# whaiproject/BetaZero

Measured on AMD Instinct MI355X. Metric: selfplay_games_per_s, higher is better.
Workload: dtype bf16

## Files before the change

betazero_amd/_lib.py:

```python
import ctypes as C
import os

HERE = os.path.dirname(os.path.abspath(__file__))
SO = os.environ.get("BZ_HIP_SO") or os.path.join(HERE, "libbz_hip.so")
ABI_VERSION = 7

BZ_OK, BZ_EINVAL, BZ_EILLEGAL_MOVE, BZ_EHIP, BZ_ENOMEM, BZ_ENOGPU, BZ_ESTATE = range(7)
GAME_TTT, GAME_REVERSI, GAME_REVERSI6, GAME_REVERSI4 = 0, 1, 2, 3
EVAL_UNIFORM, EVAL_HASH, EVAL_NET_F32, EVAL_NET_BF16, EVAL_EXTERNAL, EVAL_NET_FP8, EVAL_MLP_F32, EVAL_MLP_BF16 = range(8)
ST_RUNNING, ST_TERMINAL, ST_ILLEGAL, ST_MUST_PASS = range(4)
PASS_ACTION = 64
ENGINE_REUSE_SUBTREE = 1
ENGINE_EVAL_CACHE = 2
ENGINE_EVAL_CACHE_CARRY = 4
ENGINE_LEAVES_SHIFT = 8
ENGINE_LEAVES_MASK = 31 << ENGINE_LEAVES_SHIFT
PROBE_OPS = ("expf_spec", "logf_spec", "tanhf_spec", "fsqrt", "fdiv", "u01_spec", "hash_logit", "hash_value", "gamma_spec")
PROBE_HOST, PROBE_DEVICE = 0, 1
PROBE_MAP, PROBE_SWEEP = 0, 1
PROF_SLOTS = ("tower", "stem", "heads", "select", "expand_backup", "search_fused", "play", "env_step")
COUNTER_NAMES = ("n_sims", "n_path_nodes", "n_child_scored", "n_edges_backed", "n_expanded",
                 "n_child_written", "n_env_steps", "n_net_leaves", "n_cache_hits", "n_cache_hits_prev", "n_collisions")

u64, u32, i32, i64, vp = C.c_uint64, C.c_uint32, C.c_int32, C.c_int64, C.c_void_p
# ... 85 lines not shown
    "bz_ttt_step_batch": (i32, [vp, vp, vp, vp, i64, vp, vp, vp, vp, vp, vp]),
    "bz_reversi_minimax": (i32, [u64, u64, i32, i32, C.POINTER(i32), C.POINTER(i32)]),
    "bz_ttt_minimax": (i32, [u32, u32, i32, C.POINTER(i32), C.POINTER(i32)]),
    "bz_reversi_minimax_batch": (i32, [vp, vp, vp, i64, i32, i32, vp, vp, vp]),
    "bz_ttt_minimax_batch": (i32, [vp, vp, vp, vp, i64, vp, vp, vp]),
    "bz_augment_d4_batch": (i32, [vp, vp, vp, i64, i32, i32, vp, vp, vp, vp, vp]),
    "bz_net_update": (i32, [vp, vp, vp]),
    "bz_net_param_count": (i64, [i32, i32, i32]),
    "bz_net_workspace_bytes": (i64, [i32, i32, i32, i32]),
    "bz_net_create": (i32, [i32, i32, i32, i32, vp, vp, i64, vp, C.POINTER(vp)]),
    "bz_net_destroy": (i32, [vp]),
    "bz_net_forward_f32": (i32, [vp, vp, vp, i32, vp, vp, vp]),
    "bz_net_forward_bf16": (i32, [vp, vp, vp, i32, vp, vp, vp]),
    "bz_net_forward_fp8": (i32, [vp, vp, vp, i32, vp, vp, vp]),
    "bz_sym_index": (u32, [u64, u64, u64]),
    "bz_sym_board": (i32, [u64, i32, i32, C.POINTER(u64)]),
    "bz_sym_action_map": (i32, [i32, i32, vp]),
    "bz_net_sym_scratch_bytes": (i64, [i64]),
    "bz_net_forward_sym": (i32, [vp, i32, vp, vp, i32, i32, i32, u64, vp, i64, vp, vp, vp]),
    "bz_net_forward_sym_counted": (i32, [vp, i32, vp, vp, i32, vp, i32, i32, u64, vp, vp, vp]),
    "bz_net_forward_counted": (i32, [vp, i32, vp, vp, i32, vp, vp, vp, vp]),
    "bz_net_set_adaptive_shape": (i32, [vp, i32]),
    "bz_net_shape_tally": (i32, [vp, vp, vp]),
    "bz_mlp_param_count": (i64, [i32]),
    "bz_mlp_workspace_bytes": (i64, [i32, i32]),
    "bz_mlp_create": (i32, [i32, i32, vp, vp, i64, vp, C.POINTER(vp)]),
    "bz_mlp_destroy": (i32, [vp]),
    "bz_mlp_update": (i32, [vp, vp, vp]),
    "bz_mlp_forward_f32": (i32, [vp, vp, vp, i32, vp, vp]),
    "bz_mlp_forward_bf16": (i32, [vp, vp, vp, i32, vp, vp]),
    "bz_mlp_forward_states_f32": (i32, [vp, vp, i32, vp, vp]),
    "bz_mlp_forward_states_bf16": (i32, [vp, vp, i32, vp, vp]),
    "bz_mlp_train_workspace_bytes": (i64, [i32, i32]),
    "bz_mlp_train_step": (i32, [vp, vp, vp, vp, vp, vp, vp, vp, i32, C.POINTER(MlpAdam), vp, i64, vp, vp, vp, vp]),
    "bz_engine_workspace_bytes": (i64, [C.POINTER(EngineCfg)]),
    "bz_engine_create": (i32, [C.POINTER(EngineCfg), vp, i64, C.POINTER(vp)]),
    "bz_engine_destroy": (i32, [vp]),
    "bz_engine_get_layout": (i32, [vp, C.POINTER(EngineLayout)]),
    "bz_engine_set_net": (i32, [vp, vp]),
    "bz_engine_set_mlp": (i32, [vp, vp]),
    "bz_engine_debug_set_search_seq": (i32, [vp, C.c_uint32]),
    "bz_engine_set_eval_symmetry": (i32, [vp, i32, u64]),
    "bz_engine_reset_games": (i32, [vp, vp]),
    "bz_engine_set_roots": (i32, [vp, vp, vp, vp, vp]),
    "bz_engine_search": (i32, [vp, vp]),
    "bz_engine_root_begin": (i32, [vp, vp]),
# ... 181 lines not shown
```

betazero_amd/csrc/bz_net.hip:

```cpp
#include <limits.h>
#include <math.h>
#include <stdlib.h>
#include <new>
#include <atomic>
#include <vector>

#include "bz_common.h"
#include "bz_math.h"
#include "bz_sym.h"
#include "bz_tower.h"

using namespace bz;

using namespace bz_tower;

struct bz_net {
    int C, NB, VH, max_batch;
    float *stem_w, *stem_b;
    float *conv_w, *conv_b;
    __bf16* conv_wf;
    __bf16 *stem_wf, *head_wf;
    __bf16 *conv_wf16, *stem_wf16;
    uint8_t *conv_wf8, *head_wf8;
    float *dq8, *head_dq8, *ones;
    float *pol_w, *pol_b, *polfc_wT, *polfc_b;
    float *val_w, *val_b, *v1_wT, *v1_b, *v2_w, *v2_b;
    float *act_a, *act_b;
    void* ws_base;
    hipEvent_t f32_done;
    bool f32_used;
    int adaptive;
    uint32_t* tally;
    uint64_t epoch;
};

namespace {

#define BZ_NET_SYM 0
#include "bz_net_ends_body.h"
#undef BZ_NET_SYM
#define BZ_NET_SYM 1
#include "bz_net_ends_body.h"
#undef BZ_NET_SYM

__global__ void __launch_bounds__(256) k_conv_f32(const float* __restrict__ in, const float* __restrict__ w,
                                                  const float* __restrict__ b, const float* skip, float* out, int n,
                                                  const u32* n_dev, int C) {
    extern __shared__ __attribute__((aligned(16))) char smem_raw[];
    float* xs = reinterpret_cast<float*>(smem_raw);
    int pos = blockIdx.x;
    if (n_dev) n = (int)*n_dev;
    if (pos >= n) return;
    const float* xin = in + (size_t)pos * 64 * C;
    for (int i = threadIdx.x; i < 64 * C; i += 256) xs[i] = xin[i];
// ... 14 lines not shown
            }
            const float* wt = w + (size_t)t * C * C + co;
            for (int ci = 0; ci < C; ++ci) {
                float wv = wt[(size_t)ci * C];
#pragma unroll
                for (int j = 0; j < 8; ++j)
                    if (src[j] >= 0) acc[j] = __builtin_fmaf(xs[src[j] + ci], wv, acc[j]);
            }
        }
#pragma unroll
        for (int j = 0; j < 8; ++j) {
            size_t o = ((size_t)pos * 64 + c0 + j) * C + co;
            float v = acc[j];
            if (skip) v = v + skip[o];
            out[o] = relu_f32(v);
        }
    }
}

typedef Tw<64, 2> TwS64;
typedef Tw<128, 1> TwS128;
typedef Tw<256, 1> TwS256;
typedef Tw<128, 4, true> TwM16;
constexpr int kSmallBatch = 256;
constexpr int kAdaptT1 = 256;
enum { kShapeLatency = 0, kShapeMiddle = 1, kShapeThroughput = 2, kShapes = 4 };

struct TowerArgs {
    const u64 *own, *opp;
    const u32* n_dev;
    int n, n_layers, VH;
    int lo, hi;
    u32* tally;
    const uint4* wf;
    const uint4 *wf16, *stem_wf16;
    const float* bias;
    const uint4* stem_wf;
    const float* stem_b;
    const uint4* head_wf;
    const uint4 *wf8, *head_wf8;
    const float *dq8, *head_dq8, *ones;
    const float *pol_b, *val_b;
    const float *polfc_wT, *polfc_b;
    const float *v1_wT, *v1_b, *v2_w, *v2_b;
    float *logits, *value;
};
// ... 27 lines not shown
    unsigned wd[4];
#pragma unroll
    for (int j = 0; j < 4; ++j) {
        const int t = 4 * g + j;
        const int bit = t <= 8 ? (t / 3) * 8 + t % 3 : 31;
        const unsigned o = (n_own >> bit) & 1u, p = (n_opp >> bit) & 1u;
        wd[j] = (o | (p << 16)) * 0x3F80u;
    }
    uint4 u = make_uint4(wd[0], wd[1], wd[2], wd[3]);
    return __builtin_bit_cast(bf16x8, u);
}

__device__ __forceinline__ float wave_sum(float x) {
#pragma unroll
    for (int o = 32; o > 0; o >>= 1) x += __shfl_xor(x, o, 64);
    return x;
}

#define BZ_NET_SYM 0
#include "bz_net_tower_bf16_body.h"
#undef BZ_NET_SYM
#define BZ_NET_SYM 1
#include "bz_net_tower_bf16_body.h"
#undef BZ_NET_SYM

namespace f8 {
typedef int v8i __attribute__((ext_vector_type(8)));
typedef int v4i __attribute__((ext_vector_type(4)));
constexpr int kCell = 128, kRowC = 9;
constexpr int kTile = (8 * kRowC + 1) * kCell;
constexpr int kBuf = 4 * kTile;
constexpr int kLds = 2 * kBuf;
constexpr float kActScale = 16.0f;
constexpr int kUnit = 0x7F7F7F7F;

__device__ __forceinline__ constexpr int cell_at(int y, int x) { return (y * kRowC + x + 1) * kCell; }
__device__ __forceinline__ int sw3(int p, int x) { return ((x & 7) >> 1) | ((p & 1) << 2); }
template <int DX>
__device__ __forceinline__ int tap_off(int r, int h) {
    const int xx = (r & 7) + DX;
    return (r >> 3) * kTile + cell_at(0, xx) + (((2 * h) ^ sw3(r >> 3, xx)) << 4);
}
__device__ __forceinline__ v8i ld32(const char* p0, int off, int imm) {
    v4i lo = *reinterpret_cast<const v4i*>(p0 + off + imm);
    v4i hi = *reinterpret_cast<const v4i*>(p0 + (off ^ 16) + imm);
    v8i v = {lo[0], lo[1], lo[2], lo[3], hi[0], hi[1], hi[2], hi[3]};
// ... 381 lines not shown
BZ_EXPORT int32_t bz_net_create(int32_t C, int32_t NB, int32_t VH, int32_t max_batch, const float* p, void* ws,
                                int64_t bytes, void* stream, bz_net** out) {
    BZ_REQUIRE(shape_ok(C, NB, VH, max_batch) && p && ws && out, "bz_net_create: unsupported shape or null pointer");
    if (bz_device_count() <= 0) { set_error("bz_net_create: no HIP device (the net has no CPU path)"); return BZ_ENOGPU; }
    NetOffsets o = net_carve(C, NB, VH, max_batch);
    if (bytes < o.total) { set_error("bz_net_create: workspace too small"); return BZ_ENOMEM; }
    BZ_REQUIRE((reinterpret_cast<uintptr_t>(ws) & 255) == 0, "bz_net_create: workspace must be 256-byte aligned");
    bz_net* n = new (std::nothrow) bz_net();
    if (!n) { set_error("out of host memory"); return BZ_ENOMEM; }
    n->C = C; n->NB = NB; n->VH = VH; n->max_batch = max_batch;
    n->stem_w = at<float>(ws, o.stem_w); n->stem_b = at<float>(ws, o.stem_b);
    n->conv_w = at<float>(ws, o.conv_w); n->conv_b = at<float>(ws, o.conv_b);
    n->conv_wf = (C == 64 || C == 128 || C == 256) ? at<__bf16>(ws, o.conv_wf) : nullptr;
    n->stem_wf = at<__bf16>(ws, o.stem_wf); n->head_wf = at<__bf16>(ws, o.head_wf);
    n->conv_wf16 = C == kTC ? at<__bf16>(ws, o.conv_wf16) : nullptr; n->stem_wf16 = C == kTC ? at<__bf16>(ws, o.stem_wf16) : nullptr;
    n->conv_wf8 = C == kTC ? at<uint8_t>(ws, o.conv_wf8) : nullptr; n->head_wf8 = at<uint8_t>(ws, o.head_wf8);
    n->dq8 = at<float>(ws, o.dq8); n->head_dq8 = at<float>(ws, o.head_dq8); n->ones = at<float>(ws, o.ones);
    n->pol_w = at<float>(ws, o.pol_w); n->pol_b = at<float>(ws, o.pol_b);
    n->polfc_wT = at<float>(ws, o.polfc_wT); n->polfc_b = at<float>(ws, o.polfc_b);
    n->val_w = at<float>(ws, o.val_w); n->val_b = at<float>(ws, o.val_b);
    n->v1_wT = at<float>(ws, o.v1_wT); n->v1_b = at<float>(ws, o.v1_b);
    n->v2_w = at<float>(ws, o.v2_w); n->v2_b = at<float>(ws, o.v2_b);
    n->act_a = at<float>(ws, o.act_a); n->act_b = at<float>(ws, o.act_b);
    n->tally = at<uint32_t>(ws, o.tally); n->adaptive = 1;

    n->ws_base = ws;
    n->f32_used = false;
    if (hipEventCreateWithFlags(&n->f32_done, hipEventDisableTiming) != hipSuccess) {
        delete n; set_error("bz_net_create: hipEventCreate failed"); return BZ_EHIP;
    }
    if (hipMemsetAsync(n->tally, 0, kShapes * sizeof(uint32_t), (hipStream_t)stream) != hipSuccess) {
        (void)hipEventDestroy(n->f32_done); delete n; set_error("bz_net_create: hipMemsetAsync failed"); return BZ_EHIP;
    }
    int32_t urc = upload_params(n, p, (hipStream_t)stream);
    if (urc != BZ_OK) { delete n; return urc; }
    {
        hipError_t e3 = hipSuccess;
#define BZ_TOWER_LDS(GEOM) hipFuncSetAttribute(reinterpret_cast<const void*>(k_tower_bf16<GEOM>), hipFuncAttributeMaxDynamicSharedMemorySize, GEOM::LDS)
        if (C == 64) { e3 = BZ_TOWER_LDS(Tw<64>); if (e3 == hipSuccess) e3 = BZ_TOWER_LDS(TwS64); }
        if (C == 128) { e3 = BZ_TOWER_LDS(TwM16); if (e3 == hipSuccess) e3 = BZ_TOWER_LDS(TwS128); }
        if (C == 256) { e3 = BZ_TOWER_LDS(Tw<256>); if (e3 == hipSuccess) e3 = BZ_TOWER_LDS(TwS256); }
#undef BZ_TOWER_LDS
        if (e3 != hipSuccess) { delete n; return hip_fail(e3, "hipFuncSetAttribute(k_tower_bf16)"); }
#define BZ_TOWER_LDS(GEOM) hipFuncSetAttribute(reinterpret_cast<const void*>(k_sym_bf16<GEOM>), hipFuncAttributeMaxDynamicSharedMemorySize, GEOM::LDS)
        if (C == 64) { e3 = BZ_TOWER_LDS(Tw<64>); if (e3 == hipSuccess) e3 = BZ_TOWER_LDS(TwS64); }
        if (C == 128) { e3 = BZ_TOWER_LDS(TwM16); if (e3 == hipSuccess) e3 = BZ_TOWER_LDS(TwS128); }
        if (C == 256) { e3 = BZ_TOWER_LDS(Tw<256>); if (e3 == hipSuccess) e3 = BZ_TOWER_LDS(TwS256); }
#undef BZ_TOWER_LDS
        if (e3 != hipSuccess) { delete n; return hip_fail(e3, "hipFuncSetAttribute(k_sym_bf16)"); }
        if (C == 256) {
            e3 = hipFuncSetAttribute(reinterpret_cast<const void*>(k_heads<float>), hipFuncAttributeMaxDynamicSharedMemorySize,
                                     (int)((64 * (C + 1) + 128 + 64 + 64) * sizeof(float)));
            if (e3 == hipSuccess)
                e3 = hipFuncSetAttribute(reinterpret_cast<const void*>(k_sym_heads<float>), hipFuncAttributeMaxDynamicSharedMemorySize,
                                         (int)((64 * (C + 1) + 128 + 64 + 64) * sizeof(float)));
            if (e3 == hipSuccess)
                e3 = hipFuncSetAttribute(reinterpret_cast<const void*>(k_conv_f32), hipFuncAttributeMaxDynamicSharedMemorySize,
                                         (int)(64 * C * sizeof(float)));
            if (e3 != hipSuccess) { delete n; return hip_fail(e3, "hipFuncSetAttribute(f32 parity kernels)"); }
        }
    }
    if (C == kTC) {
        hipError_t e3 = hipFuncSetAttribute(reinterpret_cast<const void*>(f8::k_tower_fp8), hipFuncAttributeMaxDynamicSharedMemorySize,
                                 f8::kLds);
        if (e3 == hipSuccess)
            e3 = hipFuncSetAttribute(reinterpret_cast<const void*>(f8::k_sym_fp8), hipFuncAttributeMaxDynamicSharedMemorySize, f8::kLds);
        if (e3 != hipSuccess) { delete n; return hip_fail(e3, "hipFuncSetAttribute(k_tower_fp8)"); }
    }
    *out = n;
    return BZ_OK;
}

// ... 62 lines not shown
    T.dq8 = n->dq8; T.head_dq8 = n->head_dq8; T.ones = n->ones;
    T.polfc_wT = n->polfc_wT; T.polfc_b = n->polfc_b; T.v1_wT = n->v1_wT; T.v1_b = n->v1_b; T.v2_w = n->v2_w;
    T.v2_b = n->v2_b; T.logits = logits; T.value = value;
    T.lo = 0; T.hi = INT_MAX; T.tally = nullptr;
    {
        ProfScope ps(BZ_PROF_TOWER, stream);
        const bool small = cnt <= kSmallBatch;
        const bool dev128 = n_dev && !small && n->C == 128 && !fp8;
        const int mode = dev128 ? n->adaptive : 0;
        TowerArgs TS = T;
        if (dev128) T.tally = n->tally + kShapeThroughput;
        if (mode == 1) { TS.n = kAdaptT1 < cnt ? kAdaptT1 : cnt; TS.hi = kAdaptT1; TS.tally = n->tally + kShapeLatency; T.lo = kAdaptT1 + 1; }
        if (mode == 2) T.tally = n->tally + kShapeLatency;
#define BZ_TOWER_LAUNCH(KERNEL, GEOM, TA, ...) hipLaunchKernelGGL(KERNEL<GEOM>, dim3((TA.n + GEOM::P - 1) / GEOM::P), dim3(256), GEOM::LDS, s, TA, ##__VA_ARGS__)
#define BZ_TOWER_PICK(KERNEL, ...) do {                                                                               \
            if (n->C == 64) { if (small) BZ_TOWER_LAUNCH(KERNEL, TwS64, T, ##__VA_ARGS__); else BZ_TOWER_LAUNCH(KERNEL, Tw<64>, T, ##__VA_ARGS__); }        \
            else if (n->C == 256) { if (small) BZ_TOWER_LAUNCH(KERNEL, TwS256, T, ##__VA_ARGS__); else BZ_TOWER_LAUNCH(KERNEL, Tw<256>, T, ##__VA_ARGS__); } \
            else if (mode == 1) { BZ_TOWER_LAUNCH(KERNEL, TwS128, TS, ##__VA_ARGS__); BZ_TOWER_LAUNCH(KERNEL, TwM16, T, ##__VA_ARGS__); }                    \
            else { if (small || mode == 2) BZ_TOWER_LAUNCH(KERNEL, TwS128, T, ##__VA_ARGS__); else BZ_TOWER_LAUNCH(KERNEL, TwM16, T, ##__VA_ARGS__); }       \
        } while (0)
        if (fp8 && Y) hipLaunchKernelGGL(f8::k_sym_fp8, dim3((cnt + 3) / 4), dim3(256), f8::kLds, s, T, *Y);
        else if (fp8) hipLaunchKernelGGL(f8::k_tower_fp8, dim3((cnt + 3) / 4), dim3(256), f8::kLds, s, T);
        else if (Y) BZ_TOWER_PICK(k_sym_bf16, *Y);
        else BZ_TOWER_PICK(k_tower_bf16);
#undef BZ_TOWER_PICK
#undef BZ_TOWER_LAUNCH
    }
    BZ_LAUNCH_CHECK("k_tower_bf16");
    return BZ_OK;
}

BZ_EXPORT int32_t bz_net_set_adaptive_shape(bz_net* n, int32_t mode) {
    BZ_REQUIRE(n && mode >= 0 && mode <= 2, "bz_net_set_adaptive_shape: null net, or mode not 0 (off), 1 (on) or 2 (latency shape always)");
    n->adaptive = mode;
    return BZ_OK;
}
BZ_EXPORT int32_t bz_net_shape_tally(bz_net* n, int64_t* counts, void* stream) {
    BZ_REQUIRE(n && counts, "bz_net_shape_tally: null pointer");
    uint32_t h[kShapes];
    BZ_HIP(hipMemcpyAsync(h, n->tally, sizeof(h), hipMemcpyDeviceToHost, (hipStream_t)stream));
    BZ_HIP(hipMemsetAsync(n->tally, 0, sizeof(h), (hipStream_t)stream));
    BZ_HIP(hipStreamSynchronize((hipStream_t)stream));
    for (int i = 0; i < 3; ++i) counts[i] = h[i];
    return BZ_OK;
}

uint64_t bz_net_epoch(const bz_net* n) { return n ? n->epoch : 0; }
int32_t bz_net_max_batch(const bz_net* n) { return n ? n->max_batch : 0; }

int32_t bz_net_forward_dev(bz_net* n, int bf16 , const uint64_t* own, const uint64_t* opp, int32_t max_n,
                           const uint32_t* n_dev, float* logits, float* value, void* stream) {
    BZ_REQUIRE(n && own && opp && logits && value, "bz_net_forward: null pointer");
    BZ_REQUIRE(bf16 != 1 || n->C == 64 || n->C == 128 || n->C == 256,
               "bz_net_forward_bf16: the MFMA tower is built for 64, 128 or 256 channels");
    BZ_REQUIRE(bf16 != 2 || n->C == kTC, "bz_net_forward_fp8: the fp8 tower is built for C == 128");
    BZ_REQUIRE(max_n >= 0 && max_n <= n->max_batch, "bz_net_forward: batch exceeds max_batch");
    if (max_n == 0) return BZ_OK;
// ... 84 lines not shown
```

betazero_amd/csrc/bz_net_tower_bf16_body.h:

```cpp

template <class G>
__global__ void __launch_bounds__(256, 1)
#if BZ_NET_SYM
k_sym_bf16(TowerArgs T, bz_sym::Args Y) {
#else
k_tower_bf16(TowerArgs T) {
#endif
    constexpr int C = G::C, P = G::P, PW = G::PW, MW = G::MW;
    extern __shared__ __attribute__((aligned(16))) char smem[];
    const int tid = threadIdx.x, lane = tid & 63;
    const int w = __builtin_amdgcn_readfirstlane(tid >> 6);
    const int pos0 = blockIdx.x * P;
    if (T.n_dev) T.n = (int)*T.n_dev;
    if (pos0 >= T.n || T.n < T.lo || T.n > T.hi) return;
    if (T.tally && blockIdx.x == 0 && tid == 0) atomicAdd(T.tally, 1u);
    [[maybe_unused]] unsigned long long tacc[4] = {0, 0, 0, 0}, tk0 = 0, tk1 = 0, tr0 = 0, tr1 = 0;
    BZ_STAMP(tk0);
#ifdef BZ_EXP_STAMPS
    tr0 = __builtin_amdgcn_s_memrealtime();
#endif
    char* bufX = smem;
    char* bufM = smem + G::BUF;
    const int r = lane & 31, h = lane >> 5;

    constexpr int ZC = G::CELL / 16;
    for (int i = tid; i < 2 * P * 9 * ZC; i += 256) {
        int k = i % ZC, j = (i / ZC) % 9, pb = i / (9 * ZC);
        *reinterpret_cast<uint4*>(smem + pb * G::TILE + j * G::ROWC * G::CELL + k * 16) = make_uint4(0, 0, 0, 0);
    }
    const int wt0 = G::wt0(w), wp0 = G::pos0(w);
    const uint4* ap = G::M16 ? T.wf16 + (size_t)wt0 * 2 * 64 : T.wf + (size_t)wt0 * 64;
    typename WSetsOf<G>::type WS;
    if constexpr (G::M16) {
#pragma unroll
        for (int kq = 0; kq < G::KQ; ++kq)
#pragma unroll
            for (int a = 0; a < 2; ++a) WS.s[0][kq][a] = __builtin_bit_cast(bf16x8, ap[(kq * G::MT * 2 + a) * 64 + (unsigned)lane]);
        ap += G::KQ * G::MT * 2 * 64;
    } else {
#pragma unroll
        for (int d = 0; d + 1 < G::DEPTH; ++d) {
#pragma unroll
            for (int kc = 0; kc < G::KS; ++kc)
#pragma unroll
                for (int mt = 0; mt < MW; ++mt) WS.s[d][kc][mt] = __builtin_bit_cast(bf16x8, ap[(kc * G::MT + mt) * 64 + (unsigned)lane]);
            ap += G::KS * G::MT * 64;
        }
    }

    if constexpr (G::M16) {
        f32x16 acc[MW][G::NU];
        Bias<G> bias;
        const int c = lane & 15, g = lane >> 4;
        load_bias16<G>(bias, T.stem_b, wt0, g);
        bf16x8 sa[2];
#pragma unroll
        for (int a = 0; a < 2; ++a) sa[a] = __builtin_bit_cast(bf16x8, T.stem_wf16[(wt0 * 2 + a) * 64 + lane]);
        u64 own[2], opp[2];
#pragma unroll
        for (int b = 0; b < 2; ++b) {
            int pos = pos0 + wp0 + 2 * b + (c >> 3);
            pos = pos < T.n ? pos : T.n - 1;
            own[b] = T.own[pos]; opp[b] = T.opp[pos];
#if BZ_NET_SYM
            {
                const u32 s = bz_sym::of(Y, own[b], opp[b]);
                own[b] = bz_sym::board(own[b], Y.size, s); opp[b] = bz_sym::board(opp[b], Y.size, s);
            }
#endif
        }
#pragma unroll
        for (int u = 0; u < G::NU; ++u) {
            acc[0][u] = (f32x16)(0.0f);
// ... 118 lines not shown
```

betazero_amd/csrc/bz_tower.h:

```cpp
#pragma once
#include "bz_common.h"

typedef __attribute__((ext_vector_type(8))) __bf16 bf16x8;
typedef __attribute__((ext_vector_type(4))) __bf16 bf16x4;
typedef __attribute__((ext_vector_type(2))) __bf16 bf16x2;
typedef __attribute__((ext_vector_type(4))) short s16x4;
typedef __attribute__((ext_vector_type(2))) short s16x2;
typedef __attribute__((ext_vector_type(2))) float f32x2;
typedef __attribute__((ext_vector_type(4))) float f32x4;
typedef __attribute__((ext_vector_type(16))) float f32x16;

namespace bz_tower {
using namespace bz;
constexpr int kTC = 128;

template <int C_, int P_ = 512 / C_, bool M16_ = false> struct Tw {
    static_assert(C_ == 64 || C_ == 128 || C_ == 256, "the MFMA tower is built for 64, 128 or 256 channels");
    static constexpr int C = C_;
    static constexpr bool M16 = M16_;
    static constexpr int KQ = C / 32;
    static constexpr int KC = C / 16;
    static constexpr int MT = C / 32;
    static constexpr int CELL = 2 * C;
    static constexpr int ROWC = 9;
    static constexpr int NCELL = 8 * ROWC + 1;
    static constexpr int TILE = NCELL * CELL;
    static constexpr int P = P_;
    static constexpr int BUF = P * TILE;
    static constexpr int LDS = 2 * BUF;
    static constexpr int MW = MT >= 8 ? 2 : 1;
    static constexpr int PW = MT * P / 4 / MW;
    static_assert(MW * PW * 4 == MT * P && PW >= 1, "the (M-tile, position) units must split evenly over 4 waves");
    static constexpr int NG = MT / MW;
    static constexpr int NU = 2 * PW;
    static constexpr bool ROWT = PW == 4;
    static constexpr int KS = KC < 8 ? KC : 8;
    static constexpr int NBUF = 2;
    static constexpr int CPT = KC / KS;
    static constexpr int NCH = 9 * CPT;
    static constexpr int DEPTH = MW * PW <= 2 ? 3 : 2;
    static_assert((2 * NCH) % DEPTH == 0, "a residual block must bring the register-set rotation back to set 0");
    static __device__ __forceinline__ int wt0(int w) { return (w % NG) * MW; }
    static __device__ __forceinline__ int pos0(int w) { return (w / NG) * PW; }
    static __device__ __forceinline__ constexpr int cell_at(int y, int x) { return (y * ROWC + x + 1) * CELL; }
    static __device__ __forceinline__ int sw(int sel, int xx) {
        return C == 64 ? (((xx & 7) >> 1) | ((sel & 1) << 2)) : ((xx & 7) | ((sel & 1) << 3));
    }
    static __device__ __forceinline__ int pos16(int ch, int xx) {
        const int s = (ch + 2 * (xx & 7)) & 15;
        return ((s >> 1) | ((s & 1) << 3)) << 4;
    }
    static __device__ __forceinline__ int cell_off(int p, int c, int k) {
        if constexpr (M16) return cell_at(c >> 3, c & 7) + pos16(k, c & 7);
        else return cell_at(c >> 3, c & 7) + ((k ^ sw(ROWT ? p : c >> 3, c & 7)) << 4);
    }
    static __device__ __forceinline__ int unit_pos(int u, int r) { return ROWT ? r >> 3 : u >> 1; }
    static __device__ __forceinline__ int unit_cell(int u, int r) { return ROWT ? 8 * u + (r & 7) : 32 * (u & 1) + r; }
    static __device__ __forceinline__ int lane_home(int r) {
        return ROWT ? (r >> 3) * TILE + cell_at(0, r & 7) : cell_at(r >> 3, r & 7);
    }
    static __device__ __forceinline__ constexpr int unit_imm(int u) {
        return ROWT ? u * ROWC * CELL : (u >> 1) * TILE + (u & 1) * 4 * ROWC * CELL;
    }
    static __device__ __forceinline__ constexpr int unit_lo(int dy) { return ROWT && dy < 0 ? 1 : 0; }
    static __device__ __forceinline__ constexpr int unit_hi(int dy) { return ROWT && dy > 0 ? NU - 1 : NU; }
};

#ifdef BZ_EXP_STAMPS
static __device__ unsigned long long g_dbg[8 * 4096];
#define BZ_STAMP(var) do { unsigned long long _t; asm volatile("s_memtime %0\n\ts_waitcnt lgkmcnt(0)" : "=s"(_t) :: "memory"); var = _t; } while (0)
#else
#define BZ_STAMP(var) do { } while (0)
#endif

template <class G, int TAP>
__device__ __forceinline__ void tap_off(int r, int h, int (&boff)[2]) {
// ... 279 lines not shown
#pragma unroll
        for (int b = 0; b < 2; ++b)
#pragma unroll
            for (int par = 0; par < 2; ++par)
#pragma unroll
                for (int u = par; u < G::NU; u += 2) {
                    const int off = home2[par] + slot + b * 2 * G::TILE + (u & ~1) * G::ROWC * G::CELL;
                    const int q = 2 * a + b;
                    f32x4 v = {acc[0][u][4 * q], acc[0][u][4 * q + 1], acc[0][u][4 * q + 2], acc[0][u][4 * q + 3]};
                    v = v + bq;
                    if (second) {
                        bf16x4 sk = *reinterpret_cast<const bf16x4*>(out + off);
                        v = v + __builtin_convertvector(sk, f32x4);
                    }
                    v = relu_f32x4(v);
                    f32x2 vlo = {v[0], v[1]}, vhi = {v[2], v[3]};
                    s16x2 lo = __builtin_bit_cast(s16x2, __builtin_convertvector(vlo, bf16x2));
                    s16x2 hi = __builtin_bit_cast(s16x2, __builtin_convertvector(vhi, bf16x2));
                    *reinterpret_cast<uint2*>(out + off) = make_uint2(__builtin_bit_cast(unsigned, lo), __builtin_bit_cast(unsigned, hi));
                }
    }
}

template <class G> struct EpInfer {
    __device__ __forceinline__ void operator()(f32x16 (&acc)[G::MW][G::NU], char* out, bool second, const Bias<G>& bias, int wt0,
                                               int r, int h) const {
        if constexpr (G::M16) epilogue16<G>(acc, out, second, bias, wt0, 32 * h + r);
        else epilogue<G>(acc, out, second, bias, wt0, r, h);
    }
};
template <class G> struct WSetsOf { typedef WSets<G> type; };
template <int C_, int P_> struct WSetsOf<Tw<C_, P_, true>> { typedef WSets16<Tw<C_, P_, true>> type; };
template <int S0, class G, class EP = EpInfer<G>>
__device__ __forceinline__ void conv_layer(const char* in, char* out, bool second, const float* __restrict__ bl,
                                           typename WSetsOf<G>::type& WS, const uint4*& ap, int w, int r, int h,
                                           unsigned long long (&tacc)[4], const EP& ep = EP()) {
    [[maybe_unused]] unsigned long long t0 = 0, t1 = 0, t2 = 0, t3 = 0;
    BZ_STAMP(t0);
    f32x16 acc[G::MW][G::NU];
#pragma unroll
    for (int mt = 0; mt < G::MW; ++mt)
#pragma unroll
        for (int u = 0; u < G::NU; ++u) acc[mt][u] = (f32x16)(0.0f);
    const int wpos = G::pos0(w) * G::TILE;
    in += wpos; out += wpos;
    Bias<G> bias;
    if constexpr (G::M16) load_bias16<G>(bias, bl, G::wt0(w), (32 * h + r) >> 4);
    else load_bias<G>(bias, bl, G::wt0(w), h);
    int boff[2];
    if constexpr (G::M16) {
        static_assert(G::ROWT && G::MW == 1 && G::C == 128, "the 16x16x32 path serves the row-tile shape of the 128-channel net");
        bf16x8 B[2][G::NU];
        const int lane = 32 * h + r;
        int boff16[G::KQ];
        tap_off16<G, 0>(lane & 15, lane >> 4, boff16);
        load_b16<G, 0>(B[0], in, boff16[0], 0);
        __builtin_amdgcn_sched_barrier(0);
        run_taps16<S0, 0, G>(acc, WS, ap, in, boff16, lane, B);
    } else if constexpr (G::ROWT) {
        bf16x8 B[G::NBUF][G::NU];
        tap_off<G, 0>(r, h, boff);
#pragma unroll
        for (int k = 0; k + 1 < G::NBUF; ++k) load_b<G, 0>(B[k], in, boff, k);
        __builtin_amdgcn_sched_barrier(0);
        run_chunks<S0, 0, G>(acc, WS, ap, in, boff, r, h, B);
    } else {
        bf16x8 b0[G::NU], b1[G::NU];
        tap_off_pm<G>(0, r, h, boff);
        load_b<G, 4>(b0, in, boff, 0);
        auto tap_of = [](int c) { c = c < G::NCH ? c : G::NCH - 1; return c / G::CPT; };
        auto kc0_of = [](int c) { c = c < G::NCH ? c : G::NCH - 1; return (c % G::CPT) * G::KS; };
        constexpr int D = G::DEPTH, R = G::NCH % D, C0 = G::NCH - R;
#define BZ_CHUNK(J, CC) chunk_step_pm<(S0 + (J)) % D, G>(acc, WS, ap, in, boff, kc0_of(CC), tap_of((CC) + 1), kc0_of((CC) + 1), r, h, b0, b1)
// ... 20 lines not shown
```

betazero_amd/net.py:

```python
import ctypes as C

import numpy as np
import torch
import torch.nn as nn
import torch.nn.functional as F

from . import _lib


_NBHD = {}


class OwnershipHead(nn.Module):

    def __init__(self, channels=128):
        super().__init__()
        self.C = channels
        self.conv = nn.Conv2d(channels, 1, 1)

    def forward(self, x):
        return torch.tanh(self.conv(x)).flatten(1)


class PolicyValueNet(nn.Module):
# ... 142 lines not shown
    def forward_counted(self, own, opp, count, logits, value, bf16=True, fp8=False, symmetry=None, size=8, seed=0):
        from .symmetry import SYM_MEAN, check_forward_symmetry
        sym = check_forward_symmetry(symmetry, size, seed)
        if sym is not None and sym[0] == SYM_MEAN:
            raise ValueError("forward_counted: the mean over the symmetries takes a host-side count (forward)")
        n, kind = own.numel(), 2 if fp8 else (1 if bf16 else 0)
        assert opp.numel() == n and logits.shape == (n, 65) and value.shape == (n,) and count.numel() >= 1
        assert logits.dtype == value.dtype == torch.float32 and logits.is_contiguous() and count.element_size() == 4
        L = _lib.lib()
        with torch.cuda.device(self.device):
            st = torch.cuda.current_stream().cuda_stream
            if sym is None:
                _lib.check(L.bz_net_forward_counted(self.h, kind, own.data_ptr(), opp.data_ptr(), n, count.data_ptr(),
                                                    logits.data_ptr(), value.data_ptr(), st))
            else:
                _lib.check(L.bz_net_forward_sym_counted(self.h, kind, own.data_ptr(), opp.data_ptr(), n, count.data_ptr(), size,
                                                        sym[0], sym[1], logits.data_ptr(), value.data_ptr(), st))

    SHAPE_NAMES = ("latency", "middle", "throughput")

    def set_adaptive_shape(self, mode=True):
        _lib.check(_lib.lib().bz_net_set_adaptive_shape(self.h, int(mode)))

    def shape_tally(self):
        c = (C.c_int64 * 3)()
        with torch.cuda.device(self.device):
            _lib.check(_lib.lib().bz_net_shape_tally(self.h, c, torch.cuda.current_stream().cuda_stream))
        return dict(zip(self.SHAPE_NAMES, (int(v) for v in c)))

    def update(self, params):
        params = np.ascontiguousarray(params, dtype=np.float32)
        assert params.size == _lib.lib().bz_net_param_count(self.C, self.NB, self.VH)
        with torch.cuda.device(self.device):
            _lib.check(_lib.lib().bz_net_update(self.h, params.ctypes.data, torch.cuda.current_stream().cuda_stream))

    def __del__(self):
        try:
            _lib.lib().bz_net_destroy(self.h)
        except Exception:
            pass
```

include/bz_abi.h:

```cpp
#ifndef BZ_ABI_H
#define BZ_ABI_H
#include <stdint.h>

#ifdef __cplusplus
extern "C" {
#endif

#define BZ_ABI_VERSION 7

enum { BZ_OK = 0, BZ_EINVAL = 1, BZ_EILLEGAL_MOVE = 2, BZ_EHIP = 3, BZ_ENOMEM = 4, BZ_ENOGPU = 5,
       BZ_ESTATE = 6 };
enum { BZ_GAME_TTT = 0, BZ_GAME_REVERSI = 1, BZ_GAME_REVERSI6 = 2, BZ_GAME_REVERSI4 = 3 };
enum { BZ_EVAL_UNIFORM = 0, BZ_EVAL_HASH = 1, BZ_EVAL_NET_F32 = 2, BZ_EVAL_NET_BF16 = 3,
       BZ_EVAL_EXTERNAL = 4, BZ_EVAL_NET_FP8 = 5,
       BZ_EVAL_MLP_F32 = 6, BZ_EVAL_MLP_BF16 = 7 };
#define BZ_PASS_ACTION 64

int32_t bz_abi_version(void);
const char* bz_last_error(void);
const char* bz_build_info(void);
int32_t bz_device_count(void);

int32_t bz_reversi_legal(uint64_t own, uint64_t opp, int32_t size, uint64_t* legal);
int32_t bz_reversi_apply(uint64_t own, uint64_t opp, int32_t size, int32_t row, int32_t col,
// ... 28 lines not shown
int32_t bz_reversi_minimax_batch(const uint64_t* self, const uint64_t* other, const uint8_t* active, int64_t n,
                                 int32_t size, int32_t max_depth, int8_t* move, int16_t* score, void* stream);
int32_t bz_ttt_minimax_batch(const uint16_t* self, const uint16_t* other, const int8_t* symbol,
                             const uint8_t* active, int64_t n, int8_t* move, int16_t* score, void* stream);

typedef struct bz_net bz_net;
int64_t bz_net_param_count(int32_t C, int32_t NB, int32_t VH);
int64_t bz_net_workspace_bytes(int32_t C, int32_t NB, int32_t VH, int32_t max_batch);
int32_t bz_net_create(int32_t C, int32_t NB, int32_t VH, int32_t max_batch, const float* params_host,
                      void* workspace, int64_t workspace_bytes, void* stream, bz_net** out);
int32_t bz_net_destroy(bz_net* net);
int32_t bz_net_update(bz_net* net, const float* params_host, void* stream);
int32_t bz_net_forward_f32(bz_net* net, const uint64_t* own, const uint64_t* opp, int32_t n,
                           float* logits, float* value, void* stream);
int32_t bz_net_forward_bf16(bz_net* net, const uint64_t* own, const uint64_t* opp, int32_t n,
                            float* logits, float* value, void* stream);
int32_t bz_net_forward_fp8(bz_net* net, const uint64_t* own, const uint64_t* opp, int32_t n,
                           float* logits, float* value, void* stream);

int32_t bz_net_forward_counted(bz_net* net, int32_t kind, const uint64_t* own, const uint64_t* opp, int32_t max_n,
                               const uint32_t* n_dev, float* logits, float* value, void* stream);
int32_t bz_net_set_adaptive_shape(bz_net* net, int32_t mode);
int32_t bz_net_shape_tally(bz_net* net, int64_t* counts , void* stream);

uint32_t bz_sym_index(uint64_t seed, uint64_t own, uint64_t opp);
int32_t bz_sym_board(uint64_t b, int32_t size, int32_t s, uint64_t* out);
int32_t bz_sym_action_map(int32_t size, int32_t s, uint8_t* map );
enum { BZ_SYM_FIXED = 0, BZ_SYM_HASHED = 1, BZ_SYM_MEAN = 2 };
int64_t bz_net_sym_scratch_bytes(int64_t n);
int32_t bz_net_forward_sym(bz_net* net, int32_t kind, const uint64_t* own, const uint64_t* opp, int32_t n, int32_t size,
                           int32_t mode, uint64_t arg, void* scratch, int64_t scratch_bytes, float* logits, float* value,
                           void* stream);
int32_t bz_net_forward_sym_counted(bz_net* net, int32_t kind, const uint64_t* own, const uint64_t* opp, int32_t max_n,
                                   const uint32_t* n_dev, int32_t size, int32_t mode, uint64_t arg, float* logits,
                                   float* value, void* stream);

typedef struct bz_mlp bz_mlp;
int64_t bz_mlp_param_count(int32_t H);
int64_t bz_mlp_workspace_bytes(int32_t H, int32_t max_batch);
int32_t bz_mlp_create(int32_t H, int32_t max_batch, const float* params_host, void* workspace, int64_t workspace_bytes,
                      void* stream, bz_mlp** out);
int32_t bz_mlp_destroy(bz_mlp* mlp);
int32_t bz_mlp_update(bz_mlp* mlp, const float* params_host, void* stream);
int32_t bz_mlp_forward_f32(bz_mlp* mlp, const uint64_t* own, const uint64_t* opp, int32_t n, float* logits, void* stream);
int32_t bz_mlp_forward_bf16(bz_mlp* mlp, const uint64_t* own, const uint64_t* opp, int32_t n, float* logits, void* stream);
int32_t bz_mlp_forward_states_f32(bz_mlp* mlp, const float* x, int32_t n, float* logits, void* stream);
// ... 294 lines not shown
```

Baseline: 244.6.

## Add edge-aware tile map to the 128-channel bf16 tower to skip padding taps

Adds a new tower kernel variant for the 128-channel MFMA 16x16 path that maps tiles onto board edge rows, columns and interior blocks. Conv taps that fall entirely in the zero padding for edge tiles are skipped, and LDS slots are rotated to avoid bank conflicts. It is enabled by default for non-small batches, with a runtime switch to turn it off. The aim is to cut wasted MFMA work and LDS traffic on border positions, at the cost of more complex addressing and scheduling hints.

```diff
diff --git a/betazero_amd/_lib.py b/betazero_amd/_lib.py
--- a/betazero_amd/_lib.py
+++ b/betazero_amd/_lib.py
@@ -131,6 +131,7 @@
     "bz_net_forward_counted": (i32, [vp, i32, vp, vp, i32, vp, vp, vp, vp]),
     "bz_net_set_adaptive_shape": (i32, [vp, i32]),
     "bz_net_shape_tally": (i32, [vp, vp, vp]),
+    "bz_net_set_tile_map": (i32, [vp, i32]),
     "bz_mlp_param_count": (i64, [i32]),
     "bz_mlp_workspace_bytes": (i64, [i32, i32]),
     "bz_mlp_create": (i32, [i32, i32, vp, vp, i64, vp, C.POINTER(vp)]),
diff --git a/betazero_amd/csrc/bz_net.hip b/betazero_amd/csrc/bz_net.hip
--- a/betazero_amd/csrc/bz_net.hip
+++ b/betazero_amd/csrc/bz_net.hip
@@ -30,6 +30,7 @@
     hipEvent_t f32_done;
     bool f32_used;
     int adaptive;
+    int tile_map;
     uint32_t* tally;
     uint64_t epoch;
 };
@@ -90,6 +91,7 @@
 typedef Tw<128, 1> TwS128;
 typedef Tw<256, 1> TwS256;
 typedef Tw<128, 4, true> TwM16;
+typedef Tw<128, 4, true, 1> TwEdge;
 constexpr int kSmallBatch = 256;
 constexpr int kAdaptT1 = 256;
 enum { kShapeLatency = 0, kShapeMiddle = 1, kShapeThroughput = 2, kShapes = 4 };
@@ -163,6 +165,11 @@
 #undef BZ_NET_SYM
 #define BZ_NET_SYM 1
 #include "bz_net_tower_bf16_body.h"
+#undef BZ_NET_SYM
+#define BZ_NET_SYM 0
+#define BZ_NET_EDGE 1
+#include "bz_net_tower_bf16_body.h"
+#undef BZ_NET_EDGE
 #undef BZ_NET_SYM
 
 namespace f8 {
@@ -590,7 +597,7 @@
     n->v1_wT = at<float>(ws, o.v1_wT); n->v1_b = at<float>(ws, o.v1_b);
     n->v2_w = at<float>(ws, o.v2_w); n->v2_b = at<float>(ws, o.v2_b);
     n->act_a = at<float>(ws, o.act_a); n->act_b = at<float>(ws, o.act_b);
-    n->tally = at<uint32_t>(ws, o.tally); n->adaptive = 1;
+    n->tally = at<uint32_t>(ws, o.tally); n->adaptive = 1; n->tile_map = 1;
 
     n->ws_base = ws;
     n->f32_used = false;
@@ -616,6 +623,8 @@
         if (C == 256) { e3 = BZ_TOWER_LDS(Tw<256>); if (e3 == hipSuccess) e3 = BZ_TOWER_LDS(TwS256); }
 #undef BZ_TOWER_LDS
         if (e3 != hipSuccess) { delete n; return hip_fail(e3, "hipFuncSetAttribute(k_sym_bf16)"); }
+        if (C == 128) e3 = hipFuncSetAttribute(reinterpret_cast<const void*>(k_edge_bf16<TwEdge>), hipFuncAttributeMaxDynamicSharedMemorySize, TwEdge::LDS);
+        if (e3 != hipSuccess) { delete n; return hip_fail(e3, "hipFuncSetAttribute(k_edge_bf16)"); }
         if (C == 256) {
             e3 = hipFuncSetAttribute(reinterpret_cast<const void*>(k_heads<float>), hipFuncAttributeMaxDynamicSharedMemorySize,
                                      (int)((64 * (C + 1) + 128 + 64 + 64) * sizeof(float)));
@@ -724,6 +733,10 @@
         if (fp8 && Y) hipLaunchKernelGGL(f8::k_sym_fp8, dim3((cnt + 3) / 4), dim3(256), f8::kLds, s, T, *Y);
         else if (fp8) hipLaunchKernelGGL(f8::k_tower_fp8, dim3((cnt + 3) / 4), dim3(256), f8::kLds, s, T);
         else if (Y) BZ_TOWER_PICK(k_sym_bf16, *Y);
+        else if (n->C == 128 && n->tile_map && !small && mode != 2) {
+            if (mode == 1) BZ_TOWER_LAUNCH(k_tower_bf16, TwS128, TS);
+            BZ_TOWER_LAUNCH(k_edge_bf16, TwEdge, T);
+        }
         else BZ_TOWER_PICK(k_tower_bf16);
 #undef BZ_TOWER_PICK
 #undef BZ_TOWER_LAUNCH
@@ -735,6 +748,11 @@
 BZ_EXPORT int32_t bz_net_set_adaptive_shape(bz_net* n, int32_t mode) {
     BZ_REQUIRE(n && mode >= 0 && mode <= 2, "bz_net_set_adaptive_shape: null net, or mode not 0 (off), 1 (on) or 2 (latency shape always)");
     n->adaptive = mode;
+    return BZ_OK;
+}
+BZ_EXPORT int32_t bz_net_set_tile_map(bz_net* n, int32_t map) {
+    BZ_REQUIRE(n && (map == 0 || map == 1), "bz_net_set_tile_map: null net, or map not 0 (board rows) or 1 (edge-aware)");
+    n->tile_map = map;
     return BZ_OK;
 }
 BZ_EXPORT int32_t bz_net_shape_tally(bz_net* n, int64_t* counts, void* stream) {
diff --git a/betazero_amd/csrc/bz_net_tower_bf16_body.h b/betazero_amd/csrc/bz_net_tower_bf16_body.h
--- a/betazero_amd/csrc/bz_net_tower_bf16_body.h
+++ b/betazero_amd/csrc/bz_net_tower_bf16_body.h
@@ -3,6 +3,8 @@
 __global__ void __launch_bounds__(256, 1)
 #if BZ_NET_SYM
 k_sym_bf16(TowerArgs T, bz_sym::Args Y) {
+#elif BZ_NET_EDGE
+k_edge_bf16(TowerArgs T) {
 #else
 k_tower_bf16(TowerArgs T) {
 #endif
@@ -48,7 +50,38 @@
         }
     }
 
-    if constexpr (G::M16) {
+    if constexpr (G::EDGE) {
+        namespace tmap = bz_tile_map;
+        f32x16 acc[MW][G::NU];
+        Bias<G> bias;
+        const int c = lane & 15, g = lane >> 4;
+        load_bias16<G>(bias, T.stem_b, wt0, g);
+        bf16x8 sa[2];
+#pragma unroll
+        for (int a = 0; a < 2; ++a) sa[a] = __builtin_bit_cast(bf16x8, T.stem_wf16[(wt0 * 2 + a) * 64 + lane]);
+        const int lp[5] = {tmap::lane_p(tmap::kRow, c), 2 + tmap::lane_p(tmap::kRow, c), tmap::lane_p(tmap::kCol, c),
+                           tmap::lane_p(tmap::kMix, c), tmap::lane_p(tmap::kIn, c)};
+        u64 own[5], opp[5];
+#pragma unroll
+        for (int i = 0; i < 5; ++i) {
+            int pos = pos0 + wp0 + lp[i];
+            pos = pos < T.n ? pos : T.n - 1;
+            own[i] = T.own[pos]; opp[i] = T.opp[pos];
+        }
+#pragma unroll
+        for (int u = 0; u < G::NU; ++u) {
+            acc[0][u] = (f32x16)(0.0f);
+#pragma unroll
+            for (int b = 0; b < 2; ++b) {
+                const int t = 2 * u + b, i = t < 4 ? (t & 1) : 1 + tmap::pattern(t);
+                const int cell = 8 * tmap::pair_y(t, c) + tmap::pair_x(t, c);
+                const bf16x8 f = stem_frag16(nbhd(own[i], cell), nbhd(opp[i], cell), g);
+                if (b) { mfma16_quarter<1>(acc[0][u], sa[0], f); mfma16_quarter<3>(acc[0][u], sa[1], f); }
+                else { mfma16_quarter<0>(acc[0][u], sa[0], f); mfma16_quarter<2>(acc[0][u], sa[1], f); }
+            }
+        }
+        epilogue_edge<G>(acc, bufX + wp0 * G::TILE, false, bias, wt0, lane);
+    } else if constexpr (G::M16) {
         f32x16 acc[MW][G::NU];
         Bias<G> bias;
         const int c = lane & 15, g = lane >> 4;
diff --git a/betazero_amd/csrc/bz_tile_map.h b/betazero_amd/csrc/bz_tile_map.h
--- /dev/null
+++ b/betazero_amd/csrc/bz_tile_map.h
@@ -0,0 +1,53 @@
+#pragma once
+#if defined(__HIPCC__)
+#define BZ_TM_FN __host__ __device__ constexpr
+#else
+#define BZ_TM_FN constexpr
+#endif
+
+namespace bz_tile_map {
+constexpr int kTiles = 16;
+constexpr int kPairs = 16;
+constexpr int kRowC = 9;
+constexpr int kNCell = 73;
+enum { kRow = 0, kCol = 1, kMix = 2, kIn = 3, kPatterns = 4 };
+
+BZ_TM_FN int pattern(int t) { return t < 4 ? kRow : t < 6 ? kCol : t == 6 ? kMix : kIn; }
+BZ_TM_FN int tile_p(int t) { return t < 4 ? 2 * (t & 1) : 0; }
+BZ_TM_FN int tile_y(int t) { return t < 4 ? 7 * (t >> 1) : t < 6 ? 1 : t == 6 ? 5 : 1 + 2 * ((t - 7) / 3); }
+BZ_TM_FN int tile_x(int t) { return t < 5 ? 0 : t == 5 ? 7 : t == 6 ? 0 : 1 + 2 * ((t - 7) % 3); }
+BZ_TM_FN int half(int c) { return ((c + 4) >> 3) & 1; }
+BZ_TM_FN int idx(int c) { return c & 7; }
+BZ_TM_FN int lane_p(int pat, int c) {
+    return pat == kRow ? half(c) : pat == kCol ? 2 * (idx(c) >> 2) + half(c) : pat == kMix ? idx(c) & 3 : idx(c) >> 1;
+}
+BZ_TM_FN int lane_y(int pat, int c) { return pat == kRow ? 0 : pat == kCol ? idx(c) & 3 : pat == kMix ? idx(c) >> 2 : half(c); }
+BZ_TM_FN int lane_x(int pat, int c) { return pat == kRow ? idx(c) : pat == kCol ? 0 : pat == kMix ? 7 * half(c) : idx(c) & 1; }
+BZ_TM_FN int pair_p(int t, int c) { return tile_p(t) + lane_p(pattern(t), c); }
+BZ_TM_FN int pair_y(int t, int c) { return tile_y(t) + lane_y(pattern(t), c); }
+BZ_TM_FN int pair_x(int t, int c) { return tile_x(t) + lane_x(pattern(t), c); }
+BZ_TM_FN int lane_cells(int pat, int c) { return lane_p(pat, c) * kNCell + lane_y(pat, c) * kRowC + lane_x(pat, c); }
+BZ_TM_FN int tile_cells(int t) { return tile_p(t) * kNCell + tile_y(t) * kRowC + tile_x(t) + 1; }
+BZ_TM_FN int tap_cells(int tap) { return (tap / 3 - 1) * kRowC + (tap % 3 - 1); }
+BZ_TM_FN bool skip(int tap, int t) {
+    return (t < 2 && tap / 3 == 0) || (t >= 2 && t < 4 && tap / 3 == 2) || (t == 4 && tap % 3 == 0) || (t == 5 && tap % 3 == 2);
+}
+BZ_TM_FN int tiles_of_tap(int tap) {
+    int n = 0;
+    for (int t = 0; t < kTiles; ++t) n += skip(tap, t) ? 0 : 1;
+    return n;
+}
+BZ_TM_FN int tiles_of_half(int tap, int hf) {
+    int n = 0;
+    for (int t = hf; t < kTiles; t += 2) n += skip(tap, t) ? 0 : 1;
+    return n;
+}
+BZ_TM_FN int sigma(int s) { return (s >> 1) | ((s & 1) << 3); }
+BZ_TM_FN int slot(int ch, int p, int y, int x) { return sigma((ch + 2 * x + 2 * y + 4 * p) & 15); }
+BZ_TM_FN int lane_w(int pat, int c) { return lane_x(pat, c) + lane_y(pat, c) + 2 * lane_p(pat, c); }
+BZ_TM_FN int slot_rot(int t, int tap, int ch_even) {
+    return (ch_even / 2 + tile_x(t) + tile_y(t) + 2 * tile_p(t) + (tap / 3 - 1) + (tap % 3 - 1)) & 7;
+}
+BZ_TM_FN int lane_slot(int pat, int c, int sub, int rot) { return ((((sub >> 1) + lane_w(pat, c) + rot) & 7) | ((sub & 1) << 3)); }
+constexpr int kCentre = 4;
+}
diff --git a/betazero_amd/csrc/bz_tower.h b/betazero_amd/csrc/bz_tower.h
--- a/betazero_amd/csrc/bz_tower.h
+++ b/betazero_amd/csrc/bz_tower.h
@@ -1,5 +1,6 @@
 #pragma once
 #include "bz_common.h"
+#include "bz_tile_map.h"
 
 typedef __attribute__((ext_vector_type(8))) __bf16 bf16x8;
 typedef __attribute__((ext_vector_type(4))) __bf16 bf16x4;
@@ -14,9 +15,11 @@
 using namespace bz;
 constexpr int kTC = 128;
 
-template <int C_, int P_ = 512 / C_, bool M16_ = false> struct Tw {
+template <int C_, int P_ = 512 / C_, bool M16_ = false, int MAP_ = 0> struct Tw {
     static_assert(C_ == 64 || C_ == 128 || C_ == 256, "the MFMA tower is built for 64, 128 or 256 channels");
     static constexpr int C = C_;
+    static constexpr bool EDGE = MAP_ == 1;
+    static_assert(MAP_ == 0 || (MAP_ == 1 && M16_ && C_ == 128 && P_ == 4), "the edge-aware tiling serves Tw<128, 4, true> only");
     static constexpr bool M16 = M16_;
     static constexpr int KQ = C / 32;
     static constexpr int KC = C / 16;
@@ -51,7 +54,8 @@
         return ((s >> 1) | ((s & 1) << 3)) << 4;
     }
     static __device__ __forceinline__ int cell_off(int p, int c, int k) {
-        if constexpr (M16) return cell_at(c >> 3, c & 7) + pos16(k, c & 7);
+        if constexpr (EDGE) return cell_at(c >> 3, c & 7) + (bz_tile_map::slot(k, p, c >> 3, c & 7) << 4);
+        else if constexpr (M16) return cell_at(c >> 3, c & 7) + pos16(k, c & 7);
         else return cell_at(c >> 3, c & 7) + ((k ^ sw(ROWT ? p : c >> 3, c & 7)) << 4);
     }
     static __device__ __forceinline__ int unit_pos(int u, int r) { return ROWT ? r >> 3 : u >> 1; }
@@ -377,15 +381,114 @@
     }
 }
 
+namespace tmap = bz_tile_map;
+struct EdgeOff { int o[tmap::kPatterns][8]; };
+template <class G>
+__device__ __forceinline__ void edge_offsets(EdgeOff& E, int c, int sub, int rot0, int extra) {
+#pragma unroll
+    for (int pat = 0; pat < tmap::kPatterns; ++pat)
+#pragma unroll
+        for (int u = 0; u < 8; ++u)
+            E.o[pat][u] = tmap::lane_cells(pat, c) * G::CELL + (tmap::lane_slot(pat, c, sub, (u + rot0) & 7) << 4) + extra;
+}
+template <class G, int TAP>
+__device__ __forceinline__ void load_b_edge(bf16x8 (&b)[G::NU], const char* in, const EdgeOff& E, int kq, int hf) {
+#pragma unroll
+    for (int j = 0; j < G::NU; ++j) {
+        const int t = 2 * j + hf;
+        if (!tmap::skip(TAP, t))
+            b[j] = *reinterpret_cast<const bf16x8*>(in + E.o[tmap::pattern(t)][tmap::slot_rot(t, TAP, 4 * kq)] +
+                                                    (tmap::tile_cells(t) + tmap::tap_cells(TAP)) * G::CELL);
+    }
+}
+template <class G, int TAP, int HF>
+__device__ __forceinline__ void mfma_edge(f32x16 (&acc)[G::MW][G::NU], const bf16x8 (&a)[2], const bf16x8 (&b)[G::NU]) {
+#pragma unroll
+    for (int j = 0; j < G::NU; ++j)
+        if (!tmap::skip(TAP, 2 * j + HF)) {
+            mfma16_quarter<HF>(acc[0][j], a[0], b[j]);
+            mfma16_quarter<2 + HF>(acc[0][j], a[1], b[j]);
+        }
+}
+template <int S, int TAP, class G>
+__device__ __forceinline__ void tap_step_edge(f32x16 (&acc)[G::MW][G::NU], WSets16<G>& WS, const uint4*& ap, const char* in,
+                                              const EdgeOff& E, int lane, bf16x8 (&B)[2][G::NU]) {
+    constexpr bool last = TAP == 8;
+    constexpr int TAP_N = last ? TAP : TAP + 1;
+    bf16x8 (&use)[G::KQ][2] = WS.s[S];
+    bf16x8 (&nxt)[G::KQ][2] = WS.s[S ^ 1];
+#pragma unroll
+    for (int kq = 0; kq < G::KQ; ++kq)
+#pragma unroll
+        for (int a = 0; a < 2; ++a) nxt[kq][a] = __builtin_bit_cast(bf16x8, ap[(kq * G::MT * 2 + a) * 64 + (unsigned)lane]);
+    ap += G::KQ * G::MT * 2 * 64;
+    constexpr int NS = 2 * G::KQ;
+#pragma unroll
+    for (int ss = 0; ss < NS; ++ss) {
+        if (ss + 1 < NS) load_b_edge<G, TAP>(B[(ss + 1) & 1], in, E, (ss + 1) >> 1, (ss + 1) & 1);
+        else if constexpr (!last) load_b_edge<G, TAP_N>(B[0], in, E, 0, 0);
+        if (ss & 1) mfma_edge<G, TAP, 1>(acc, use[ss >> 1], B[1]);
+        else mfma_edge<G, TAP, 0>(acc, use[ss >> 1], B[0]);
+    }
+#pragma unroll
+    for (int i = 0; i < NS; ++i) {
+        const int nm = tmap::tiles_of_half(TAP, i & 1);
+        const int nr = i + 1 < NS ? tmap::tiles_of_half(TAP, (i + 1) & 1) : last ? 0 : tmap::tiles_of_half(TAP_N, 0);
+#pragma unroll
+        for (int j = 0; j < G::NU; ++j) {
+            if (j < nm) __builtin_amdgcn_sched_group_barrier(0x008, 2, 0);
+            if (j < nr) __builtin_amdgcn_sched_group_barrier(0x100, 1, 0);
+        }
+        __builtin_amdgcn_sched_group_barrier(0x020, 1, 0);
+    }
+    __builtin_amdgcn_sched_barrier(0);
+}
+template <int S0, int TAP, class G>
+__device__ __forceinline__ void run_taps_edge(f32x16 (&acc)[G::MW][G::NU], WSets16<G>& WS, const uint4*& ap, const char* in,
+                                              const EdgeOff& E, int lane, bf16x8 (&B)[2][G::NU]) {
+    if constexpr (TAP < 9) {
+        tap_step_edge<(S0 + TAP) & 1, TAP, G>(acc, WS, ap, in, E, lane, B);
+        run_taps_edge<S0, TAP + 1, G>(acc, WS, ap, in, E, lane, B);
+    }
+}
+template <class G>
+__device__ __forceinline__ void epilogue_edge(f32x16 (&acc)[G::MW][G::NU], char* out, bool second, const Bias<G>& bias, int wt,
+                                              int lane) {
+    const int c = lane & 15, g = lane >> 4;
+    EdgeOff E;
+    edge_offsets<G>(E, c, g >> 1, 2 * wt, 8 * (g & 1));
+#pragma unroll
+    for (int a = 0; a < 2; ++a) {
+        const f32x4 bq = bias.q[0][a];
+#pragma unroll
+        for (int t = 0; t < tmap::kTiles; ++t) {
+            const int off = E.o[tmap::pattern(t)][tmap::slot_rot(t, tmap::kCentre, 2 * a)] + tmap::tile_cells(t) * G::CELL;
+            const int q = 2 * a + (t & 1), u = t >> 1;
+            f32x4 v = {acc[0][u][4 * q], acc[0][u][4 * q + 1], acc[0][u][4 * q + 2], acc[0][u][4 * q + 3]};
+            v = v + bq;
+            if (second) {
+                bf16x4 sk = *reinterpret_cast<const bf16x4*>(out + off);
+                v = v + __builtin_convertvector(sk, f32x4);
+            }
+            v = relu_f32x4(v);
+            f32x2 vlo = {v[0], v[1]}, vhi = {v[2], v[3]};
+            s16x2 lo = __builtin_bit_cast(s16x2, __builtin_convertvector(vlo, bf16x2));
+            s16x2 hi = __builtin_bit_cast(s16x2, __builtin_convertvector(vhi, bf16x2));
+            *reinterpret_cast<uint2*>(out + off) = make_uint2(__builtin_bit_cast(unsigned, lo), __builtin_bit_cast(unsigned, hi));
+        }
+    }
+}
+
 template <class G> struct EpInfer {
     __device__ __forceinline__ void operator()(f32x16 (&acc)[G::MW][G::NU], char* out, bool second, const Bias<G>& bias, int wt0,
                                                int r, int h) const {
-        if constexpr (G::M16) epilogue16<G>(acc, out, second, bias, wt0, 32 * h + r);
+        if constexpr (G::EDGE) epilogue_edge<G>(acc, out, second, bias, wt0, 32 * h + r);
+        else if constexpr (G::M16) epilogue16<G>(acc, out, second, bias, wt0, 32 * h + r);
         else epilogue<G>(acc, out, second, bias, wt0, r, h);
     }
 };
 template <class G> struct WSetsOf { typedef WSets<G> type; };
-template <int C_, int P_> struct WSetsOf<Tw<C_, P_, true>> { typedef WSets16<Tw<C_, P_, true>> type; };
+template <int C_, int P_, int MAP_> struct WSetsOf<Tw<C_, P_, true, MAP_>> { typedef WSets16<Tw<C_, P_, true, MAP_>> type; };
 template <int S0, class G, class EP = EpInfer<G>>
 __device__ __forceinline__ void conv_layer(const char* in, char* out, bool second, const float* __restrict__ bl,
                                            typename WSetsOf<G>::type& WS, const uint4*& ap, int w, int r, int h,
@@ -403,7 +506,15 @@
     if constexpr (G::M16) load_bias16<G>(bias, bl, G::wt0(w), (32 * h + r) >> 4);
     else load_bias<G>(bias, bl, G::wt0(w), h);
     int boff[2];
-    if constexpr (G::M16) {
+    if constexpr (G::EDGE) {
+        bf16x8 B[2][G::NU];
+        const int lane = 32 * h + r;
+        EdgeOff E;
+        edge_offsets<G>(E, lane & 15, lane >> 4, 0, 0);
+        load_b_edge<G, 0>(B[0], in, E, 0, 0);
+        __builtin_amdgcn_sched_barrier(0);
+        run_taps_edge<S0, 0, G>(acc, WS, ap, in, E, lane, B);
+    } else if constexpr (G::M16) {
         static_assert(G::ROWT && G::MW == 1 && G::C == 128, "the 16x16x32 path serves the row-tile shape of the 128-channel net");
         bf16x8 B[2][G::NU];
         const int lane = 32 * h + r;
diff --git a/betazero_amd/net.py b/betazero_amd/net.py
--- a/betazero_amd/net.py
+++ b/betazero_amd/net.py
@@ -188,6 +188,9 @@
     def set_adaptive_shape(self, mode=True):
         _lib.check(_lib.lib().bz_net_set_adaptive_shape(self.h, int(mode)))
 
+    def set_tile_map(self, edge=True):
+        _lib.check(_lib.lib().bz_net_set_tile_map(self.h, int(edge)))
+
     def shape_tally(self):
         c = (C.c_int64 * 3)()
         with torch.cuda.device(self.device):
diff --git a/include/bz_abi.h b/include/bz_abi.h
--- a/include/bz_abi.h
+++ b/include/bz_abi.h
@@ -74,6 +74,7 @@
                                const uint32_t* n_dev, float* logits, float* value, void* stream);
 int32_t bz_net_set_adaptive_shape(bz_net* net, int32_t mode);
 int32_t bz_net_shape_tally(bz_net* net, int64_t* counts , void* stream);
+int32_t bz_net_set_tile_map(bz_net* net, int32_t map);
 
 uint32_t bz_sym_index(uint64_t seed, uint64_t own, uint64_t opp);
 int32_t bz_sym_board(uint64_t b, int32_t size, int32_t s, uint64_t* out);
```

Result: faster. 250.2, median of 6 (+2.3%).
